# pearsonlab/autoencoded-vocal-analysis

Hardware: AMD Instinct MI355X
Metric: spectrograms/sec, VAE train step (fwd+bwd+Adam), 128x128, batch 256 per GPU (higher is better)
Workload: dtype f32 (fc1/fc8 products, the forward convolutions with >= 8 input channels and the fused backward kernels (data gradient AND weight gradient): fp32 operands as three bf16 limbs on bf16 MFMA, six limb products, fp32 accumulate; the 1<->8-channel layers, convt6's forward, conv7's forward and the small f; 1 GPU; configs[1]: mouse_sylls VAE, batch 256 synthetic 128x128 fp32 spectrograms per GPU, z=32, train step = zero_grad+forward+backward+Adam, device-resident batches; global_batch=256, per_gpu_batch=256, z_dim=32, parallelism=dp1

## Files before the change

autoencoded-vocal-analysis_amd/csrc/gemm_limb.hip:

```cpp
#include <type_traits>
#include "gemm.h"

typedef __bf16 bf16x8 __attribute__((ext_vector_type(8)));
typedef __bf16 bf16x2 __attribute__((ext_vector_type(2)));
typedef float f32x2 __attribute__((ext_vector_type(2)));
typedef float f32x4 __attribute__((ext_vector_type(4)));
typedef uint32_t u32x4 __attribute__((ext_vector_type(4)));
typedef uint32_t u32x2 __attribute__((ext_vector_type(2)));

#define LBK 32

__device__ __forceinline__ float limb_sub(float a, float b) {
  float r;
  asm("v_sub_f32 %0, %1, %2" : "=v"(r) : "v"(a), "v"(b));
  return r;
}
__device__ __forceinline__ void limb_split2(float x, float y, uint32_t& p0, uint32_t& p1, uint32_t& p2) {
  p0 = __builtin_bit_cast(uint32_t, __builtin_convertvector((f32x2){x, y}, bf16x2));
  float rx = limb_sub(x, __uint_as_float(p0 << 16)), ry = limb_sub(y, __uint_as_float(p0 & 0xffff0000u));
  p1 = __builtin_bit_cast(uint32_t, __builtin_convertvector((f32x2){rx, ry}, bf16x2));
  rx = limb_sub(rx, __uint_as_float(p1 << 16));
  ry = limb_sub(ry, __uint_as_float(p1 & 0xffff0000u));
  p2 = __builtin_bit_cast(uint32_t, __builtin_convertvector((f32x2){rx, ry}, bf16x2));
}

template <bool PERM>
__device__ __forceinline__ int pos16(int r) {
  return PERM ? ((r & ~5) | ((r & 1) << 2) | ((r >> 2) & 1)) : r;
}
template <bool PERM>
__device__ __forceinline__ int chunk_of(int r, int oct) {
  return PERM ? (oct ^ ((r & 1) << 1)) : (oct ^ ((4 - ((r >> 2) & 3)) & 3));
}


template <int BT, int T, int LIMB_RING>
struct LimbLoaderK {
  static constexpr int UNITS = BT * 4, NU = (UNITS + T - 1) / T;
  float4 r[LIMB_RING][NU][2];
  unsigned ok[LIMB_RING];
  size_t off[NU];
  unsigned okrow;
  __device__ __forceinline__ void init(int t0, int extent, int ld) {
    okrow = 0u;
#pragma unroll
    for (int i = 0; i < NU; ++i) {
      const int u = threadIdx.x + T * i, row = u >> 2, oct = u & 3, g = t0 + row;
      if (u < UNITS && g < extent) okrow |= 1u << i;
      off[i] = (size_t)min(g, extent - 1) * ld + oct * 8;
    }
  }
  template <int SLOT>
  __device__ __forceinline__ void load(const float* __restrict__ base, int , int k0, int kend, int K) {
    unsigned okk = 0u;
#pragma unroll
    for (int i = 0; i < NU; ++i) {
      const int oct = (threadIdx.x + T * i) & 3, gk = k0 + oct * 8;
      const float* p = base + off[i] + min(k0, K - 8 - oct * 8);
      r[SLOT][i][0] = *reinterpret_cast<const float4*>(p);
      r[SLOT][i][1] = *reinterpret_cast<const float4*>(p + 4);
      if (gk < kend) okk |= 1u << i;
    }
    ok[SLOT] = okk & okrow;
  }
  template <int SLOT, bool COLSUM>
  __device__ __forceinline__ void store(unsigned char* __restrict__ S) {
#pragma unroll
    for (int i = 0; i < NU; ++i) {
      const int u = threadIdx.x + T * i, row = u >> 2, oct = u & 3;
      if (UNITS % T != 0 && u >= UNITS) continue;
      float4 a = r[SLOT][i][0], b = r[SLOT][i][1];
      if (!((ok[SLOT] >> i) & 1u)) { a = make_float4(0.f, 0.f, 0.f, 0.f); b = a; }
      u32x4 p0, p1, p2;
      uint32_t x, y, z;
      limb_split2(a.x, a.y, x, y, z); p0[0] = x; p1[0] = y; p2[0] = z;
      limb_split2(a.z, a.w, x, y, z); p0[1] = x; p1[1] = y; p2[1] = z;
      limb_split2(b.x, b.y, x, y, z); p0[2] = x; p1[2] = y; p2[2] = z;
      limb_split2(b.z, b.w, x, y, z); p0[3] = x; p1[3] = y; p2[3] = z;
      unsigned char* d = S + row * 64 + chunk_of<false>(row & 15, oct) * 16;
      *reinterpret_cast<u32x4*>(d) = p0;
      *reinterpret_cast<u32x4*>(d + BT * 64) = p1;
      *reinterpret_cast<u32x4*>(d + 2 * BT * 64) = p2;
    }
  }
};

template <int BT, int T, int LIMB_RING>
struct LimbLoaderN {
  static constexpr int KPU = (2 * BT >= T) ? 4 : 2;
  static constexpr int KQ = LBK / KPU;
  static constexpr int UNITS = (BT / 4) * KQ, NU = (UNITS + T - 1) / T;
  float4 r[LIMB_RING][NU][KPU];
  unsigned ok[LIMB_RING];
  int coff[NU];
  unsigned okcol;
  float cs[NU][4];
  __device__ __forceinline__ LimbLoaderN() {
#pragma unroll
    for (int i = 0; i < NU; ++i)
#pragma unroll
      for (int c = 0; c < 4; ++c) cs[i][c] = 0.f;
  }
  __device__ __forceinline__ void init(int t0, int extent, int ) {
    okcol = 0u;
#pragma unroll
    for (int i = 0; i < NU; ++i) {
      const int u = threadIdx.x + T * i, cq = u / KQ, g = t0 + 4 * cq;
      if (u < UNITS && g < extent) okcol |= ((1u << KPU) - 1u) << (KPU * i);
      coff[i] = min(g, extent - 4);
    }
  }
  template <int SLOT>
  __device__ __forceinline__ void load(const float* __restrict__ base, int ld, int k0, int kend, int K) {
    unsigned okk = 0u;
#pragma unroll
    for (int i = 0; i < NU; ++i) {
      const int kq = (threadIdx.x + T * i) % KQ;
#pragma unroll
      for (int j = 0; j < KPU; ++j) {
        const int gk = k0 + KPU * kq + j;
        r[SLOT][i][j] = *reinterpret_cast<const float4*>(base + (size_t)min(gk, K - 1) * ld + coff[i]);
        if (gk < kend) okk |= 1u << (KPU * i + j);
      }
    }
    ok[SLOT] = okk & okcol;
  }
  template <int SLOT, bool COLSUM>
  __device__ __forceinline__ void store(unsigned char* __restrict__ S) {
#pragma unroll
    for (int i = 0; i < NU; ++i) {
      const int u = threadIdx.x + T * i, kq = u % KQ, cq = u / KQ;
      if (UNITS % T != 0 && u >= UNITS) continue;
      float v[KPU][4];
#pragma unroll
      for (int j = 0; j < KPU; ++j) {
        const bool okj = (ok[SLOT] >> (KPU * i + j)) & 1u;
        v[j][0] = okj ? r[SLOT][i][j].x : 0.f; v[j][1] = okj ? r[SLOT][i][j].y : 0.f;
        v[j][2] = okj ? r[SLOT][i][j].z : 0.f; v[j][3] = okj ? r[SLOT][i][j].w : 0.f;
      }
#pragma unroll
      for (int c = 0; c < 4; ++c) {
        const int row = 4 * cq + c;
        unsigned char* d = S + ((row & ~15) + pos16<true>(row & 15)) * 64;
        uint32_t x, y, z;
        if constexpr (KPU == 4) {
          if (COLSUM) cs[i][c] += (v[0][c] + v[1][c]) + (v[2][c] + v[3][c]);
          u32x2 p0, p1, p2;
          limb_split2(v[0][c], v[1][c], x, y, z); p0[0] = x; p1[0] = y; p2[0] = z;
          limb_split2(v[2][c], v[3][c], x, y, z); p0[1] = x; p1[1] = y; p2[1] = z;
          d += chunk_of<true>(row & 15, kq >> 1) * 16 + (kq & 1) * 8;
          *reinterpret_cast<u32x2*>(d) = p0;
          *reinterpret_cast<u32x2*>(d + BT * 64) = p1;
          *reinterpret_cast<u32x2*>(d + 2 * BT * 64) = p2;
        } else {
          if (COLSUM) cs[i][c] += v[0][c] + v[1][c];
          limb_split2(v[0][c], v[1][c], x, y, z);
          d += chunk_of<true>(row & 15, kq >> 2) * 16 + (kq & 3) * 4;
          *reinterpret_cast<uint32_t*>(d) = x;
          *reinterpret_cast<uint32_t*>(d + BT * 64) = y;
          *reinterpret_cast<uint32_t*>(d + 2 * BT * 64) = z;
        }
      }
    }
  }
};

template <int BT, int T, int RING, bool KMAJ>
struct LimbLoader;
template <int BT, int T, int RING>
struct LimbLoader<BT, T, RING, true> : LimbLoaderK<BT, T, RING> {};
template <int BT, int T, int RING>
struct LimbLoader<BT, T, RING, false> : LimbLoaderN<BT, T, RING> {};

template <int J, int R, class F>
__device__ __forceinline__ void limb_for_stage(F&& f) {
  f(std::integral_constant<int, J>{});
  if constexpr (J + 1 < R) limb_for_stage<J + 1, R>(f);
}

struct LimbItem { int m0, n0, split, kbeg, kend, bx; };

template <int BN, bool A_KMAJ, bool B_KMAJ, int RING, int MINW>
__global__ __launch_bounds__(512, MINW) void gemm_limb_kernel(const GemmArgs g, const int tiles_m, const int tiles_n,
                                                              const int nitems) {
  constexpr int NSW = 4;
  constexpr int BM = 128, T = 64 * NSW, WM = BM / 2, WN = BN / 2, TM = WM / 16, TN = WN / 16;
  constexpr int A_BYTES = 3 * BM * 64, B_BYTES = 3 * BN * 64, BUF = A_BYTES + B_BYTES;
  __shared__ __align__(16) unsigned char smem[2 * BUF];

  const int t = threadIdx.x, lane = t & 63, wave8 = t >> 6;
  const bool stager = wave8 < NSW;
  int it, it_end, it_step;
  {
    const int gsz = (int)gridDim.x, w = (int)blockIdx.x;
    if (((gsz | nitems) & 7) == 0) { const int chunk = nitems >> 3, x = w & 7; it = x * chunk + (w >> 3); it_end = (x + 1) * chunk; it_step = gsz >> 3; }
    else { it = w; it_end = nitems; it_step = gsz; }
  }
  auto decode = [&](int item) __attribute__((always_inline)) {
    LimbItem r;
    const int per = tiles_m * tiles_n;
    r.split = item / per;
    const int rem = item - r.split * per;
    const int by = rem / tiles_n;
    r.bx = rem - by * tiles_n;
    r.m0 = by * BM; r.n0 = r.bx * BN;
    r.kbeg = r.split * g.klen;
    r.kend = min(g.K, r.kbeg + g.klen);
    return r;
  };
  if (it >= it_end) return;

  if (stager) {
    __builtin_amdgcn_s_setprio(3);
    LimbLoader<BM, T, RING, A_KMAJ> la;
    LimbLoader<BN, T, RING, B_KMAJ> lb;
    int S = 0;
    for (int i = it; i < it_end; i += it_step) { const LimbItem q = decode(i); S += (q.kend - q.kbeg + LBK - 1) / LBK; }
    int l_it = it, s_it = it;
    LimbItem li = decode(l_it), si = li;
    int l_k = li.kbeg, s_k = si.kbeg;
    auto load_step = [&](auto slot) __attribute__((always_inline)) {
      constexpr int SLOT = decltype(slot)::value;
      if (l_k == li.kbeg) { la.init(li.m0, g.M, g.lda); lb.init(li.n0, g.N, g.ldb); }
      la.template load<SLOT>(g.A, g.lda, l_k, li.kend, g.K);
      lb.template load<SLOT>(g.B, g.ldb, l_k, li.kend, g.K);
      l_k += LBK;
      if (l_k >= li.kend) {
        l_it += it_step;
        if (l_it < it_end) { li = decode(l_it); l_k = li.kbeg; }
      }
    };
    auto store_step = [&](auto slot, int buf) __attribute__((always_inline)) {
      constexpr int SLOT = decltype(slot)::value;
      unsigned char* S_ = smem + buf * BUF;
      la.template store<SLOT, !A_KMAJ>(S_);
      lb.template store<SLOT, false>(S_ + A_BYTES);
      s_k += LBK;
      if (s_k >= si.kend) {
        if constexpr (!A_KMAJ) {
          if (g.colsum != nullptr && si.bx == 0) {
            const bool fin = g.splits == 1;
#pragma unroll
            for (int i = 0; i < LimbLoaderN<BM, T, RING>::NU; ++i) {
              constexpr int KQA = LimbLoaderN<BM, T, RING>::KQ;
              const int u = t + T * i, cq = u / KQA;
#pragma unroll
              for (int c = 0; c < 4; ++c) {
                float v = la.cs[i][c];
#pragma unroll
                for (int o = 1; o < KQA; o <<= 1) v += __shfl_xor(v, o, 64);
                const int gm = si.m0 + 4 * cq + c;
                if ((u % KQA) == 0 && u < LimbLoaderN<BM, T, RING>::UNITS && gm < g.M) {
                  if (fin) g.colsum[gm] = v;
                  else g.C[(size_t)g.splits * g.M * g.N + (size_t)si.split * g.M + gm] = v;
                }
              }
            }
          }
#pragma unroll
          for (int i = 0; i < LimbLoaderN<BM, T, RING>::NU; ++i)
#pragma unroll
            for (int c = 0; c < 4; ++c) la.cs[i][c] = 0.f;
        }
        s_it += it_step;
        if (s_it < it_end) { si = decode(s_it); s_k = si.kbeg; }
      }
    };
    limb_for_stage<0, RING - 1>([&](auto J) __attribute__((always_inline)) { if (decltype(J)::value < S) load_step(J); });
    store_step(std::integral_constant<int, 0>{}, 0);
    __syncthreads();
    int s0 = 0;
    for (; s0 + 2 * RING - 2 < S; s0 += RING)
      limb_for_stage<0, RING>([&](auto J) __attribute__((always_inline)) {
        constexpr int j = decltype(J)::value;
        load_step(std::integral_constant<int, (j + RING - 1) % RING>{});
        store_step(std::integral_constant<int, (j + 1) % RING>{}, (s0 + j + 1) & 1);
        __syncthreads();
      });
    for (; s0 < S; s0 += RING)
      limb_for_stage<0, RING>([&](auto J) __attribute__((always_inline)) {
        constexpr int j = decltype(J)::value;
        if (s0 + j < S) {
          if (s0 + j + RING - 1 < S) load_step(std::integral_constant<int, (j + RING - 1) % RING>{});
          if (s0 + j + 1 < S) store_step(std::integral_constant<int, (j + 1) % RING>{}, (s0 + j + 1) & 1);
          __syncthreads();
        }
      });
    return;
  }

  const int wave = wave8 - NSW, wm = wave >> 1, wn = wave & 1;
  const int fr = lane & 15, kg = lane >> 4;
  const int a_lane = (wm * WM) * 64 + pos16<!A_KMAJ>(fr) * 64 + chunk_of<!A_KMAJ>(fr, kg) * 16;
  const int b_lane = A_BYTES + (wn * WN) * 64 + pos16<!B_KMAJ>(fr) * 64 + chunk_of<!B_KMAJ>(fr, kg) * 16;
  f32x4 acc[TM][TN];
  __syncthreads();
  int s = 0;
  for (; it < it_end; it += it_step) {
    const LimbItem ci = decode(it);
#pragma unroll
    for (int i = 0; i < TM; ++i)
#pragma unroll
      for (int j = 0; j < TN; ++j) acc[i][j] = (f32x4){0.f, 0.f, 0.f, 0.f};
    for (int k0 = ci.kbeg; k0 < ci.kend; k0 += LBK, ++s) {
      const unsigned char* As = smem + (s & 1) * BUF + a_lane;
      const unsigned char* Bs = smem + (s & 1) * BUF + b_lane;
      bf16x8 af[TM][3];
#pragma unroll
      for (int i = 0; i < TM; ++i)
#pragma unroll
        for (int l = 0; l < 3; ++l) af[i][l] = *reinterpret_cast<const bf16x8*>(As + l * BM * 64 + i * 1024);
#pragma unroll
      for (int j = 0; j < TN; ++j) {
        bf16x8 bf[3];
#pragma unroll
        for (int l = 0; l < 3; ++l) bf[l] = *reinterpret_cast<const bf16x8*>(Bs + l * BN * 64 + j * 1024);
#pragma unroll
        for (int i = 0; i < TM; ++i) acc[i][j] = __builtin_amdgcn_mfma_f32_16x16x32_bf16(bf[0], af[i][2], acc[i][j], 0, 0, 0);
#pragma unroll
        for (int i = 0; i < TM; ++i) acc[i][j] = __builtin_amdgcn_mfma_f32_16x16x32_bf16(bf[2], af[i][0], acc[i][j], 0, 0, 0);
#pragma unroll
        for (int i = 0; i < TM; ++i) acc[i][j] = __builtin_amdgcn_mfma_f32_16x16x32_bf16(bf[1], af[i][1], acc[i][j], 0, 0, 0);
#pragma unroll
        for (int i = 0; i < TM; ++i) acc[i][j] = __builtin_amdgcn_mfma_f32_16x16x32_bf16(bf[0], af[i][1], acc[i][j], 0, 0, 0);
#pragma unroll
        for (int i = 0; i < TM; ++i) acc[i][j] = __builtin_amdgcn_mfma_f32_16x16x32_bf16(bf[1], af[i][0], acc[i][j], 0, 0, 0);
#pragma unroll
        for (int i = 0; i < TM; ++i) acc[i][j] = __builtin_amdgcn_mfma_f32_16x16x32_bf16(bf[0], af[i][0], acc[i][j], 0, 0, 0);
      }
      __syncthreads();
    }
    const bool fin = g.splits == 1;
    const int ldo = fin ? g.ldc : g.N;
    float* __restrict__ obase = fin ? g.C : g.C + (size_t)ci.split * g.M * g.N;
    const bool plain = !fin || (g.bias == nullptr && g.mask == nullptr && g.act == ACT_NONE);
    const bool relu = g.act == ACT_RELU;
    if (plain) {
#pragma unroll
      for (int i = 0; i < TM; ++i) {
        const int gm = ci.m0 + wm * WM + i * 16 + fr;
        if (gm >= g.M) continue;
#pragma unroll
        for (int j = 0; j < TN; ++j) {
          const int gn = ci.n0 + wn * WN + j * 16 + 4 * kg;
          if (gn >= g.N) continue;
          *reinterpret_cast<f32x4*>(obase + (size_t)gm * ldo + gn) = acc[i][j];
        }
      }
    } else {
      float4 bq[TN];
#pragma unroll
      for (int j = 0; j < TN; ++j) {
        const int gn = ci.n0 + wn * WN + j * 16 + 4 * kg;
        bq[j] = make_float4(0.f, 0.f, 0.f, 0.f);
        if (g.bias != nullptr && gn < g.N) bq[j] = *reinterpret_cast<const float4*>(g.bias + gn);
      }
#pragma unroll
      for (int i = 0; i < TM; ++i) {
        const int gm = ci.m0 + wm * WM + i * 16 + fr;
        if (gm >= g.M) continue;
#pragma unroll
        for (int j = 0; j < TN; ++j) {
          const int gn = ci.n0 + wn * WN + j * 16 + 4 * kg;
          if (gn >= g.N) continue;
          float cv[4] = {acc[i][j][0], acc[i][j][1], acc[i][j][2], acc[i][j][3]};
          cv[0] += bq[j].x; cv[1] += bq[j].y; cv[2] += bq[j].z; cv[3] += bq[j].w;
          if (relu) { cv[0] = fmaxf(cv[0], 0.f); cv[1] = fmaxf(cv[1], 0.f); cv[2] = fmaxf(cv[2], 0.f); cv[3] = fmaxf(cv[3], 0.f); }
          if (g.mask != nullptr) {
            const float4 mk = *reinterpret_cast<const float4*>(g.mask + (size_t)gm * g.ldc + gn);
            if (!(mk.x > 0.f)) cv[0] = 0.f;
            if (!(mk.y > 0.f)) cv[1] = 0.f;
            if (!(mk.z > 0.f)) cv[2] = 0.f;
            if (!(mk.w > 0.f)) cv[3] = 0.f;
          }
          *reinterpret_cast<float4*>(obase + (size_t)gm * ldo + gn) = make_float4(cv[0], cv[1], cv[2], cv[3]);
        }
      }
    }
  }
}

static bool limb_shape(int M, int N, int K) {
  const int mn = M < N ? M : N, mnk = mn < K ? mn : K;
  const size_t pair = (size_t)M * N * K / (size_t)mnk;
  return pair >= ((size_t)1 << 22);
}

bool ava_gemm_limb_ok(const GemmArgs& g, int a_kmajor, int b_kmajor) {
  if (!limb_shape(g.M, g.N, g.K) || !g.vec_a || !g.vec_b) return false;
  if ((a_kmajor || b_kmajor) && g.K % 8 != 0) return false;
  if (!a_kmajor && g.M % 4 != 0) return false;
  if (!b_kmajor && g.N % 4 != 0) return false;
  if (g.colsum != nullptr && a_kmajor) return false;
  if (g.act != ACT_NONE && g.act != ACT_RELU) return false;
  if (g.N % 4 != 0 || g.ldc % 4 != 0 || (reinterpret_cast<uintptr_t>(g.C) & 15) != 0) return false;
  if (g.bias != nullptr && (reinterpret_cast<uintptr_t>(g.bias) & 15) != 0) return false;
  if (g.mask != nullptr && (reinterpret_cast<uintptr_t>(g.mask) & 15) != 0) return false;
  return true;
}

void ava_gemm_limb_plan(int M, int N, int K, int a_kmajor, int* bn, int* splits, int* klen) {
  const int b = a_kmajor ? 64 : 128;
  const int tiles = ceil_div(M, 128) * ceil_div(N, b);
  const int want = b == 64 ? 512 : 256;
  int s = 1;
  if (tiles < want * 3 / 4) {
    s = ceil_div(want, tiles);
    const int max_s = K / 64 > 0 ? K / 64 : 1;
    if (s > max_s) s = max_s;
  }
  int kl = ceil_div(ceil_div(K, s), LBK) * LBK;
  s = ceil_div(K, kl);
  *bn = b; *splits = s; *klen = kl;
}

int ava_gemm_limb_launch(const GemmArgs& g, int a_kmajor, int b_kmajor, int bn, hipStream_t st) {
  const int tm = ceil_div(g.M, 128), tn = ceil_div(g.N, bn), nitems = tm * tn * g.splits;
  static int cus = 0;
  if (cus == 0) {
    int dev = 0;
    hipDeviceProp_t prop;
    cus = (hipGetDevice(&dev) == hipSuccess && hipGetDeviceProperties(&prop, dev) == hipSuccess && prop.multiProcessorCount > 0)
              ? prop.multiProcessorCount : 256;
  }
  const int resident = ava_scale_grid((bn == 64 ? 2 : 1) * cus);
  int grid = nitems < resident ? nitems : resident;
  if (bn == 64 && a_kmajor) {
    if (b_kmajor) hipLaunchKernelGGL((gemm_limb_kernel<64, true, true, 3, 4>), dim3(grid), dim3(512), 0, st, g, tm, tn, nitems);
    else hipLaunchKernelGGL((gemm_limb_kernel<64, true, false, 3, 4>), dim3(grid), dim3(512), 0, st, g, tm, tn, nitems);
  } else if (bn == 128 && !a_kmajor) {
    if (b_kmajor) hipLaunchKernelGGL((gemm_limb_kernel<128, false, true, 4, 2>), dim3(grid), dim3(512), 0, st, g, tm, tn, nitems);
    else hipLaunchKernelGGL((gemm_limb_kernel<128, false, false, 4, 2>), dim3(grid), dim3(512), 0, st, g, tm, tn, nitems);
  }
  else return AVA_EINVAL;
  AVA_CHECK_LAUNCH();
  return AVA_OK;
}
```

Before: 183,600 spectrograms/s.

## Add 256x128 limb GEMM tile with held-B fragment order for large M

Generalizes the limb GEMM kernel over BM, WM and staging-wave count, and dispatches a 256x128 tile with 128-row warp tiles when M exceeds 128 on the non-k-major A path. For large warp tiles it holds the B fragments in registers and streams A, which reduces LDS fragment reads per MFMA. The larger tile raises register pressure and shared memory use and produces fewer work items, so occupancy and load balance may suffer on mid-sized GEMMs.

After: 185,000 spectrograms/s, median of 6. No clear change (+0.8%).

```diff
diff --git a/autoencoded-vocal-analysis_amd/csrc/gemm_limb.hip b/autoencoded-vocal-analysis_amd/csrc/gemm_limb.hip
--- a/autoencoded-vocal-analysis_amd/csrc/gemm_limb.hip
+++ b/autoencoded-vocal-analysis_amd/csrc/gemm_limb.hip
@@ -180,11 +180,12 @@
 
 struct LimbItem { int m0, n0, split, kbeg, kend, bx; };
 
-template <int BN, bool A_KMAJ, bool B_KMAJ, int RING, int MINW>
-__global__ __launch_bounds__(512, MINW) void gemm_limb_kernel(const GemmArgs g, const int tiles_m, const int tiles_n,
-                                                              const int nitems) {
-  constexpr int NSW = 4;
-  constexpr int BM = 128, T = 64 * NSW, WM = BM / 2, WN = BN / 2, TM = WM / 16, TN = WN / 16;
+template <int BM, int BN, int WM, int NSW, bool A_KMAJ, bool B_KMAJ, int RING, int MINW>
+__global__ __launch_bounds__(64 * (NSW + 2 * (BM / WM)), MINW) void gemm_limb_kernel(const GemmArgs g, const int tiles_m,
+                                                                                     const int tiles_n, const int nitems) {
+  constexpr int T = 64 * NSW;
+  static_assert(T <= 4 * BN, "every staging thread needs a unit of the B tile");
+  constexpr int WN = BN / 2, TM = WM / 16, TN = WN / 16;
   constexpr int A_BYTES = 3 * BM * 64, B_BYTES = 3 * BN * 64, BUF = A_BYTES + B_BYTES;
   __shared__ __align__(16) unsigned char smem[2 * BUF];
 
@@ -305,28 +306,33 @@
     for (int k0 = ci.kbeg; k0 < ci.kend; k0 += LBK, ++s) {
       const unsigned char* As = smem + (s & 1) * BUF + a_lane;
       const unsigned char* Bs = smem + (s & 1) * BUF + b_lane;
-      bf16x8 af[TM][3];
-#pragma unroll
-      for (int i = 0; i < TM; ++i)
-#pragma unroll
-        for (int l = 0; l < 3; ++l) af[i][l] = *reinterpret_cast<const bf16x8*>(As + l * BM * 64 + i * 1024);
-#pragma unroll
-      for (int j = 0; j < TN; ++j) {
-        bf16x8 bf[3];
-#pragma unroll
-        for (int l = 0; l < 3; ++l) bf[l] = *reinterpret_cast<const bf16x8*>(Bs + l * BN * 64 + j * 1024);
-#pragma unroll
-        for (int i = 0; i < TM; ++i) acc[i][j] = __builtin_amdgcn_mfma_f32_16x16x32_bf16(bf[0], af[i][2], acc[i][j], 0, 0, 0);
-#pragma unroll
-        for (int i = 0; i < TM; ++i) acc[i][j] = __builtin_amdgcn_mfma_f32_16x16x32_bf16(bf[2], af[i][0], acc[i][j], 0, 0, 0);
-#pragma unroll
-        for (int i = 0; i < TM; ++i) acc[i][j] = __builtin_amdgcn_mfma_f32_16x16x32_bf16(bf[1], af[i][1], acc[i][j], 0, 0, 0);
-#pragma unroll
-        for (int i = 0; i < TM; ++i) acc[i][j] = __builtin_amdgcn_mfma_f32_16x16x32_bf16(bf[0], af[i][1], acc[i][j], 0, 0, 0);
-#pragma unroll
-        for (int i = 0; i < TM; ++i) acc[i][j] = __builtin_amdgcn_mfma_f32_16x16x32_bf16(bf[1], af[i][0], acc[i][j], 0, 0, 0);
-#pragma unroll
-        for (int i = 0; i < TM; ++i) acc[i][j] = __builtin_amdgcn_mfma_f32_16x16x32_bf16(bf[0], af[i][0], acc[i][j], 0, 0, 0);
+      constexpr bool HOLD_B = TM > 4 && TN >= 4;
+      constexpr int NH = HOLD_B ? TN : TM, NS = HOLD_B ? TM : TN;
+      const unsigned char* Hs = HOLD_B ? Bs : As;
+      const unsigned char* Ss = HOLD_B ? As : Bs;
+      constexpr int HP = (HOLD_B ? BN : BM) * 64, SP = (HOLD_B ? BM : BN) * 64;
+      bf16x8 hf[NH][3];
+#pragma unroll
+      for (int i = 0; i < NH; ++i)
+#pragma unroll
+        for (int l = 0; l < 3; ++l) hf[i][l] = *reinterpret_cast<const bf16x8*>(Hs + l * HP + i * 1024);
+#pragma unroll
+      for (int j = 0; j < NS; ++j) {
+        bf16x8 sf[3];
+#pragma unroll
+        for (int l = 0; l < 3; ++l) sf[l] = *reinterpret_cast<const bf16x8*>(Ss + l * SP + j * 1024);
+        auto pair = [&](auto LB_, auto LA_) __attribute__((always_inline)) {
+          constexpr int lb = decltype(LB_)::value, la = decltype(LA_)::value;
+#pragma unroll
+          for (int i = 0; i < NH; ++i) {
+            if constexpr (HOLD_B) acc[j][i] = __builtin_amdgcn_mfma_f32_16x16x32_bf16(hf[i][lb], sf[la], acc[j][i], 0, 0, 0);
+            else acc[i][j] = __builtin_amdgcn_mfma_f32_16x16x32_bf16(sf[lb], hf[i][la], acc[i][j], 0, 0, 0);
+          }
+        };
+        using I0 = std::integral_constant<int, 0>;
+        using I1 = std::integral_constant<int, 1>;
+        using I2 = std::integral_constant<int, 2>;
+        pair(I0{}, I2{}); pair(I2{}, I0{}); pair(I1{}, I1{}); pair(I0{}, I1{}); pair(I1{}, I0{}); pair(I0{}, I0{});
       }
       __syncthreads();
     }
@@ -414,8 +420,9 @@
   *bn = b; *splits = s; *klen = kl;
 }
 
-int ava_gemm_limb_launch(const GemmArgs& g, int a_kmajor, int b_kmajor, int bn, hipStream_t st) {
-  const int tm = ceil_div(g.M, 128), tn = ceil_div(g.N, bn), nitems = tm * tn * g.splits;
+template <int BM, int BN, int WM, int NSW, bool A_KMAJ, bool B_KMAJ, int RING, int MINW>
+static void limb_launch(const GemmArgs& g, int per_cu, hipStream_t st) {
+  const int tm = ceil_div(g.M, BM), tn = ceil_div(g.N, BN), nitems = tm * tn * g.splits;
   static int cus = 0;
   if (cus == 0) {
     int dev = 0;
@@ -423,14 +430,24 @@
     cus = (hipGetDevice(&dev) == hipSuccess && hipGetDeviceProperties(&prop, dev) == hipSuccess && prop.multiProcessorCount > 0)
               ? prop.multiProcessorCount : 256;
   }
-  const int resident = ava_scale_grid((bn == 64 ? 2 : 1) * cus);
-  int grid = nitems < resident ? nitems : resident;
+  const int resident = ava_scale_grid(per_cu * cus);
+  const int grid = nitems < resident ? nitems : resident;
+  hipLaunchKernelGGL((gemm_limb_kernel<BM, BN, WM, NSW, A_KMAJ, B_KMAJ, RING, MINW>), dim3(grid),
+                     dim3(64 * (NSW + 2 * (BM / WM))), 0, st, g, tm, tn, nitems);
+}
+
+int ava_gemm_limb_launch(const GemmArgs& g, int a_kmajor, int b_kmajor, int bn, hipStream_t st) {
   if (bn == 64 && a_kmajor) {
-    if (b_kmajor) hipLaunchKernelGGL((gemm_limb_kernel<64, true, true, 3, 4>), dim3(grid), dim3(512), 0, st, g, tm, tn, nitems);
-    else hipLaunchKernelGGL((gemm_limb_kernel<64, true, false, 3, 4>), dim3(grid), dim3(512), 0, st, g, tm, tn, nitems);
+    if (b_kmajor) limb_launch<128, 64, 64, 4, true, true, 3, 4>(g, 2, st);
+    else limb_launch<128, 64, 64, 4, true, false, 3, 4>(g, 2, st);
   } else if (bn == 128 && !a_kmajor) {
-    if (b_kmajor) hipLaunchKernelGGL((gemm_limb_kernel<128, false, true, 4, 2>), dim3(grid), dim3(512), 0, st, g, tm, tn, nitems);
-    else hipLaunchKernelGGL((gemm_limb_kernel<128, false, false, 4, 2>), dim3(grid), dim3(512), 0, st, g, tm, tn, nitems);
+    if (g.M > 128) {
+      if (b_kmajor) limb_launch<256, 128, 128, 4, false, true, 3, 2>(g, 1, st);
+      else limb_launch<256, 128, 128, 4, false, false, 3, 2>(g, 1, st);
+    } else {
+      if (b_kmajor) limb_launch<128, 128, 64, 4, false, true, 4, 2>(g, 1, st);
+      else limb_launch<128, 128, 64, 4, false, false, 4, 2>(g, 1, st);
+    }
   }
   else return AVA_EINVAL;
   AVA_CHECK_LAUNCH();
```
